# halajun/diasss

Hardware: AMD Instinct MI355X
Metric: sonar frames/sec end-to-end (extract+match+LM solve) (higher is better)
Workload: dtype u8/int32 (extract, match) + f64 (geo gate, LM); 1 GPU; 200 synthetic 2000x1024 frames, dense all-pairs; frames=200, pings=2000, bins=1024, pairs=19900

## Files before the change

### diasss_amd/csrc/dsss_ctx.hip

```cpp
#include "dsss_internal.h"
#include "dsss_pg_sym.h"
#include <algorithm>
#include <chrono>
#include <thread>
#include <atomic>
#include <cstdlib>

void dsss_prof_flush(dsss_ctx* c)
{
    if (!c || c->prof.pending.empty()) return;
    hipStreamSynchronize(c->stream);
    for (const dsss_prof::rec& r : c->prof.pending) {
        float ms = 0;
        if (hipEventElapsedTime(&ms, r.e0, r.e1) == hipSuccess) { c->prof.ms[r.k] += ms; c->prof.launches[r.k] += r.nl; }
        c->prof.pool.push_back(r.e0); c->prof.pool.push_back(r.e1);
    }
    c->prof.pending.clear();
}

dsss_switches dsss_switches_read()
{
    dsss_switches sw;
    if (const char* v = getenv("DSSS_EX_SCRATCH_MB")) sw.ex_scratch_mb = (size_t)std::max(1, atoi(v));
    if (const char* v = getenv("DSSS_EX_UPLOAD_BATCH")) sw.ex_upload_batch = std::max(1, atoi(v));
    sw.ex_verbose = getenv("DSSS_EX_VERBOSE") != nullptr;
    if (const char* v = getenv("DSSS_FS_THREADS")) sw.fs_threads = atoi(v);
    if (const char* v = getenv("DSSS_MT_GRID")) sw.mt_grid = atoi(v) != 0;
    sw.sift_hist_dump = getenv("DSSS_SIFT_HIST_DUMP");
    if (const char* v = getenv("DSSS_REG_PEAKS")) sw.reg_peaks_host = strcmp(v, "host") == 0;
    return sw;
}

extern "C" {

void dsss_mask_params_default(dsss_mask_params* p) { p->factor = 2.5; p->width = 10; p->r = 6; p->side = 150; }
void dsss_orb_params_default(dsss_orb_params* p) { p->nfeatures = 2000; p->scale = 1.2f; p->nlevels = 6; p->ini_th = 12; p->min_th = 7; p->descriptor = DSSS_DESC_ORB; }
void dsss_match_params_default(dsss_match_params* p)
{
    p->use_l2 = 0; p->radius = 8; p->bound_same = 88; p->bound_diff = 80; p->l2_bound = 350; p->ratio = 0.35;
    p->scc_iters = 1000; p->pix_err = 2.5; p->merge_thr = 2.5;
}
void dsss_pg_params_default(dsss_pg_params* p)
{
    p->max_iters = 100; p->rel_tol = 1e-5; p->abs_tol = 1e-5; p->lambda0 = 1e-5; p->lambda_factor = 10;
    p->lambda_max = 1e5; p->min_fidelity = 1e-3; p->add_noise = 1;
}

const char* dsss_strerror(int code)
{
    switch (code) {
    case DSSS_OK: return "ok";
    case DSSS_E_NODEVICE: return "no HIP device (libdsss has no CPU fallback)";
    case DSSS_E_ARG: return "bad argument";
    case DSSS_E_HIP: return "HIP runtime error";
    case DSSS_E_STATE: return "call order violated";
    case DSSS_E_CAPACITY: return "buffer too small";
    case DSSS_E_NUMERIC: return "numerical failure";
    case DSSS_E_COMM: return "communicator / RCCL failure";
    default: return "unknown error";
    }
}
const char* dsss_last_error(const dsss_ctx* c) { return c ? c->err.c_str() : "null context"; }

static int kcap_for(const dsss_orb_params& op) { return ((op.nfeatures + 3 * op.nlevels + 63) / 64 + 1) * 64; }

int dsss_create(int device, int max_frames, dsss_ctx** out)
{
    if (!out || max_frames <= 0) return DSSS_E_ARG;
    int ndev = 0;
    if (hipGetDeviceCount(&ndev) != hipSuccess || ndev <= 0 || device < 0 || device >= ndev) return DSSS_E_NODEVICE;
    if (hipSetDevice(device) != hipSuccess) return DSSS_E_NODEVICE;
    dsss_ctx* c = new dsss_ctx();
    c->device = device;
    dsss_mask_params_default(&c->mp); dsss_orb_params_default(&c->op);
    dsss_match_params_default(&c->mt); dsss_pg_params_default(&c->pg);
    c->max_frames = max_frames;
    c->frames.resize(max_frames);
    c->kcap = kcap_for(c->op);
    if (hipStreamCreateWithFlags(&c->stream, hipStreamNonBlocking) != hipSuccess) { delete c; return DSSS_E_HIP; }
    hipEventCreate(&c->prof.e0); hipEventCreate(&c->prof.e1);
    int prio_lo = 0, prio_hi = 0;
    (void)hipDeviceGetStreamPriorityRange(&prio_lo, &prio_hi);
    for (int i = 0; i < 4; ++i) {
        if (i == 1 && prio_hi != prio_lo) { if (hipStreamCreateWithPriority(&c->xs[i], hipStreamNonBlocking, prio_hi) != hipSuccess) { (void)hipGetLastError(); c->xs[i] = nullptr; } }
        if (!c->xs[i]) hipStreamCreateWithFlags(&c->xs[i], hipStreamNonBlocking);
        hipEventCreateWithFlags(&c->xev[i], hipEventDisableTiming);
    }
    for (int i = 0; i < DSSS_MAX_LEVELS; ++i) { hipEventCreateWithFlags(&c->ex_lev_ev[i], hipEventDisableTiming); hipEventCreateWithFlags(&c->ex_cmp_ev[i], hipEventDisableTiming); }
    for (int i = 0; i < 3; ++i) hipEventCreateWithFlags(&c->ex_side_ev[i], hipEventDisableTiming);
    hipEventCreateWithFlags(&c->xev_main, hipEventDisableTiming);
    *out = c;
    return DSSS_OK;
}

static std::array<dsss_fam_slot, 2> pack_family(dsss_frame& f, size_t pack = 0) { return {{ dsss_slot(f.d_pack, pack * sizeof(double)), dsss_slot(f.h_pack, pack * sizeof(double), DSSS_PINNED) }}; }
static std::array<dsss_fam_slot, 2> gbatch_family(dsss_geo_batch& G, size_t total = 0) { return {{ dsss_slot(G.d, total * sizeof(double)), dsss_slot(G.h, total * sizeof(double), DSSS_PINNED) }}; }
static std::array<dsss_fam_slot, 7> store_family(dsss_ctx* c)
{
    const size_t F = (size_t)c->max_frames, K = (size_t)c->kcap;
    return {{ dsss_slot(c->kps, F * K * sizeof(dsss_kp)), dsss_slot(c->desc, F * K * 32), dsss_slot(c->geo, F * K * 2 * sizeof(double)), dsss_slot(c->nkp_dev, F * sizeof(int)),
              dsss_slot(c->rows_dev, F * sizeof(int)), dsss_slot(c->cols_dev, F * sizeof(int)), dsss_slot(c->bbox_dev, F * 4 * sizeof(double)) }};
}

static void free_frame(dsss_frame& f)
{
    dsss_family_release(f.pack_cap, pack_family(f));
    hipFree(f.mask);
    if (f.pack_ev) hipEventDestroy(f.pack_ev);
    for (int l = 0; l < DSSS_MAX_LEVELS; ++l) hipFree(f.lvl[l]);
    f = dsss_frame();
}

// ... 712 lines not shown
```

### diasss_amd/csrc/dsss_internal.h

```cpp
#pragma once
#include <hip/hip_runtime.h>
#include <cstdint>
#include <cstdio>
#include <cstring>
#include <cmath>
#include <cassert>
#include <array>
#include <string>
#include <utility>
#include <vector>
#include "../../include/dsss.h"

#define DSSS_MAX_LEVELS 8
#define DSSS_PI_REF 3.14159265359

struct dsss_ctx;
int dsss_hip_fail(dsss_ctx* c, hipError_t e, const char* file, int line, const char* call);
int dsss_alloc_fail(dsss_ctx* c, hipError_t e, const char* name, const char* step, size_t bytes);

inline hipError_t dsss_mem_alloc(void** p, size_t bytes, bool pinned) { return pinned ? hipHostMalloc(p, bytes, hipHostMallocDefault) : hipMalloc(p, bytes); }
inline void dsss_mem_free(void* p, bool pinned) { if (p) { if (pinned) (void)hipHostFree(p); else (void)hipFree(p); } }

struct dsss_buf {
    void* p = nullptr; size_t cap = 0; const char* const name; const bool pinned;
// ... 137 lines not shown
    dsss_prof prof;
};

#define DSSS_FAIL(ctx, code, ...) do { char _b[512]; snprintf(_b, sizeof _b, __VA_ARGS__); (ctx)->err = _b; return (code); } while (0)
#define HIPCHK(ctx, call) do { hipError_t _e = (call); if (_e != hipSuccess) return dsss_hip_fail((ctx), _e, __FILE__, __LINE__, #call); } while (0)
inline int dsss_hip_fail(dsss_ctx* c, hipError_t e, const char* file, int line, const char* call)
{
    char b[512]; snprintf(b, sizeof b, "%s:%d %s -> %s", file, line, call, hipGetErrorString(e));
    c->err = b; return DSSS_E_HIP;
}

inline int dsss_alloc_fail(dsss_ctx* c, hipError_t e, const char* name, const char* step, size_t bytes)
{
    char b[512]; snprintf(b, sizeof b, "%s: %s (%zu bytes) -> %s", name, step, bytes, hipGetErrorString(e));
    c->err = b; return DSSS_E_HIP;
}

inline int dsss_buf::reserve(dsss_ctx* c, size_t need_bytes, size_t alloc_bytes)
{
    if (cap >= need_bytes) return DSSS_OK;
    hipError_t e = p ? hipStreamSynchronize(c->stream) : hipSuccess;
    if (e != hipSuccess) { release(); return dsss_alloc_fail(c, e, name, "hipStreamSynchronize before the old block goes", alloc_bytes); }
    release();
    void* q = nullptr;
    if ((e = dsss_mem_alloc(&q, alloc_bytes, pinned)) != hipSuccess) return dsss_alloc_fail(c, e, name, pinned ? "hipHostMalloc" : "hipMalloc", alloc_bytes);
    p = q; cap = alloc_bytes;
    return DSSS_OK;
}
inline int dsss_buf::reserve_keep(dsss_ctx* c, size_t need_bytes, size_t alloc_bytes, size_t keep_bytes)
{
    if (cap >= need_bytes) return DSSS_OK;
    hipError_t e = p ? hipStreamSynchronize(c->stream) : hipSuccess;
    if (e != hipSuccess) return dsss_alloc_fail(c, e, name, "hipStreamSynchronize before the old block goes", alloc_bytes);
    dsss_buf nw(name, pinned);
    if ((e = dsss_mem_alloc(&nw.p, alloc_bytes, pinned)) != hipSuccess) { nw.p = nullptr; return dsss_alloc_fail(c, e, name, pinned ? "hipHostMalloc" : "hipMalloc", alloc_bytes); }
    nw.cap = alloc_bytes;
    if (keep_bytes > 0 && p && (e = hipMemcpy(nw.p, p, keep_bytes, hipMemcpyDeviceToDevice)) != hipSuccess) return dsss_alloc_fail(c, e, name, "copy of the kept prefix", keep_bytes);
    *this = std::move(nw);
    return DSSS_OK;
}
template <class Fam> int dsss_family_alloc(dsss_ctx* c, const char* name, size_t& cap, size_t new_cap, const Fam& fam)
{
    bool any = false;
    for (const dsss_fam_slot& s : fam) any = any || *s.pp != nullptr;
    hipError_t e = any ? hipStreamSynchronize(c->stream) : hipSuccess;
    dsss_family_release(cap, fam);
    if (e != hipSuccess) return dsss_alloc_fail(c, e, name, "hipStreamSynchronize before the old blocks go", 0);
    for (const dsss_fam_slot& s : fam) {
        void* q = nullptr;
        if ((e = dsss_mem_alloc(&q, s.bytes, s.pinned)) != hipSuccess) { dsss_family_release(cap, fam); return dsss_alloc_fail(c, e, name, s.pinned ? "hipHostMalloc" : "hipMalloc", s.bytes); }
        *s.pp = q;
    }
    cap = new_cap;
    return DSSS_OK;
}

struct dsss_scope {
    dsss_ctx* c; int k; int nl; hipEvent_t e0 = nullptr, e1 = nullptr;
    static hipEvent_t take(dsss_ctx* c) {
        hipEvent_t e = nullptr;
        if (!c->prof.pool.empty()) { e = c->prof.pool.back(); c->prof.pool.pop_back(); } else hipEventCreate(&e);
        return e;
    }
    dsss_scope(dsss_ctx* c_, int k_, double work = 0, int launches = 1) : c(c_), k(k_), nl(launches) {
        if (c->prof.on) { c->prof.work[k] += work; e0 = take(c); e1 = take(c); hipEventRecord(e0, c->stream); }
    }
    ~dsss_scope() {
        if (e0) {
            hipEventRecord(e1, c->stream);
            c->prof.pending.push_back({ k, nl, e0, e1 });
            if (c->prof.pending.size() >= 16384) dsss_prof_flush(c);
        }
    }
};

struct dsss_switches {
    size_t ex_scratch_mb = 24576;
    int ex_upload_batch = 8;
    bool ex_verbose = false;
    int fs_threads = 0;
    bool mt_grid = true;
    const char* sift_hist_dump = nullptr;
    bool reg_peaks_host = false;
};
dsss_switches dsss_switches_read();

void dsss_extract_eager(dsss_ctx* c, const int* ids, int n, const dsss_switches& sw);
int dsss_ensure_store(dsss_ctx* c);
int dsss_ensure_sift_store(dsss_ctx* c);
struct ex_frame;
void dsss_launch_sift_desc(dsss_ctx* c, hipStream_t st, const ex_frame* d_exf, int kcap, int nb, const char* hist_dump);
int dsss_frame_geo_bbox(dsss_ctx* c, int id);
int dsss_bboxes_enqueue(dsss_ctx* c);
int dsss_sync_bboxes(dsss_ctx* c);
int dsss_frame_kp_geo(dsss_ctx* c, int id, int n);
int dsss_mt_reserve_pair_index(dsss_ctx* c, size_t npairs);
int dsss_mt_reserve_pair_match(dsss_ctx* c, size_t npairs);
int dsss_mt_reserve_rows(dsss_ctx* c, size_t n);
int dsss_mt_upload_ptr_tables(dsss_ctx* c);
void dsss_mt_clear_results(dsss_ctx* c);
void dsss_mt_free(dsss_ctx* c);
void dsss_pg_free(dsss_ctx* c);
void dsss_comm_free(dsss_ctx* c);
int dsss_comm_rank(const dsss_ctx* c);
int dsss_comm_world(const dsss_ctx* c);
int dsss_comm_allreduce(dsss_ctx* c, double* dev, size_t n, hipStream_t st);
int dsss_comm_allgather(dsss_ctx* c, void* recv_dev, size_t bytes_per_rank, hipStream_t st);

__host__ __device__ inline void dsss_sincos(double x, double* s, double* c)
{
    const double invpio2 = 6.36619772367581382433e-01;
    const double pio2_1 = 1.57079632673412561417e+00;
    const double pio2_1t = 6.07710050650619224932e-11;
    double k = rint(x * invpio2);
    double r = (x - k * pio2_1) - k * pio2_1t;
    double z = r * r;
    double ps = 1.58969099521155010221e-10;
    ps = ps * z + -2.50507602534068634195e-08;
    ps = ps * z + 2.75573137070700676789e-06;
    ps = ps * z + -1.98412698298579493134e-04;
    ps = ps * z + 8.33333333332248946124e-03;
    ps = ps * z + -1.66666666666666324348e-01;
    double sr = r + (r * z) * ps;
    double pc = -1.13596475577881948265e-11;
    pc = pc * z + 2.08757232129817482790e-09;
    pc = pc * z + -2.75573143513906633035e-07;
    pc = pc * z + 2.48015872894767294178e-05;
    pc = pc * z + -1.38888888888741095749e-03;
    pc = pc * z + 4.16666666666666019037e-02;
    double cr = (1.0 - 0.5 * z) + (z * z) * pc;
    long long q = ((long long)k) & 3;
    if (q == 0) { *s = sr; *c = cr; }
    else if (q == 1) { *s = cr; *c = -sr; }
    else if (q == 2) { *s = -sr; *c = -cr; }
    else { *s = -cr; *c = sr; }
}

__host__ __device__ inline void dsss_geo_side(const double* P, bool starboard, double* s, double* c)
{
    dsss_sincos(starboard ? P[2] + DSSS_PI_REF / 2 : P[2] - DSSS_PI_REF / 2, s, c);
}
__host__ __device__ inline int dsss_geo_index(int M, int col)
{
    int half = M / 2, idx;
    if (col >= half) idx = col - half;
    else { idx = half - col; if (idx > half - 1) idx = half - 1; }
    return idx;
}
__host__ __device__ inline void dsss_geo_bin(const double* P, const double* gr, int M, int col, double s, double c, double* x, double* y)
{
    const int idx = dsss_geo_index(M, col);
    *x = (P[3] - 0.0) + gr[idx] * c;
    *y = (P[4] - 0.0) + gr[idx] * s;
}
__host__ __device__ inline void dsss_geo_at(const double* pose6, const double* gr, int M, int row, int col,
                                            double* x, double* y)
{
    const double* P = pose6 + (size_t)row * 6;
    double s, c;
    dsss_geo_side(P, col >= M / 2, &s, &c);
    dsss_geo_bin(P, gr, M, col, s, c, x, y);
}
__host__ __device__ inline void dsss_rotate_row(const double* row, double cx, double cy, double theta, double s, double c, double* out)
{
    out[0] = row[0]; out[1] = row[1]; out[5] = row[5];
    if (theta == 0.0) { out[2] = row[2]; out[3] = row[3]; out[4] = row[4]; return; }
// ... 7 lines not shown
```

### diasss_amd/csrc/dsss_lc.hip

```cpp
#include "dsss_internal.h"
#include "dsss_pose.h"
#include "dsss_lm.h"
#include <algorithm>

#define MR 16
#define MD 15

struct mini_prob {
    pose_t prior, odo;
    double sig_prior[6], sig_odo[6], sig_s[2], sig_t[2];
    double slant_s, slant_t;
};
struct mini_val { double L[3]; pose_t X1, X2; };

#define LG 16
#define LS 16
#define LIDX(i, k) ((k) * LS + (i) + 1)
struct lc_lds { double J[MR * LS]; double H[MD * LS]; double r[MR]; mini_prob m; mini_val v, nv; };

__device__ inline void lc_bcast_pose(const pose_t& mine, int src, pose_t* out)
{
#pragma unroll
    for (int k = 0; k < 9; ++k) out->R[k] = __shfl(mine.R[k], src, LG);
#pragma unroll
    for (int k = 0; k < 3; ++k) out->t[k] = __shfl(mine.t[k], src, LG);
}
__device__ inline void lc_select_pose(bool second, const pose_t& a, const pose_t& b, pose_t* out)
{
#pragma unroll
    for (int k = 0; k < 9; ++k) out->R[k] = second ? b.R[k] : a.R[k];
#pragma unroll
    for (int k = 0; k < 3; ++k) out->t[k] = second ? b.t[k] : a.t[k];
}
__device__ static void mini_lin(const mini_prob& m, const mini_val& v, double* r, double* J, int lane)
{
    const bool hb = (lane & 8) != 0;
    const bool wr = J && (lane & 7) == 0;
    if (J) {
#pragma unroll
        for (int c2 = 0; c2 < LS; ++c2) J[lane * LS + c2] = 0.0;
        __builtin_amdgcn_wave_barrier();
    }
    pose_t t1, t2, E; double xi[6], rr[6];
    const pose_t* P = hb ? &v.X1 : &m.prior;
    const pose_t* Q = hb ? &v.X2 : &v.X1;
    pose_between(P, Q, &t1);
    pose_between(&m.odo, &t1, &t2);
    lc_select_pose(hb, t1, t2, &E);
    pose_log(&E, xi);
#pragma unroll
    for (int i = 0; i < 6; ++i) { const double sg = hb ? m.sig_odo[i] : m.sig_prior[i]; rr[i] = xi[i] / sg; }
    if (!J) {
#pragma unroll
        for (int i = 0; i < 6; ++i) { r[i] = __shfl(rr[i], 0, LG); r[6 + i] = __shfl(rr[i], 8, LG); }
    } else if (wr) {
#pragma unroll
        for (int i = 0; i < 6; ++i) r[(hb ? 6 : 0) + i] = rr[i];
    }
    if (J) {
        pose_t hi; double Ad[36];
        pose_inverse(&t1, &hi);
        pose_adjoint(&hi, Ad);
        if (wr && !hb) {
#pragma unroll
            for (int i = 0; i < 6; ++i) J[i * LS + 3 + i] = 1.0 / m.sig_prior[i];
        }
        if (wr && hb) {
#pragma unroll
            for (int i = 0; i < 6; ++i) {
#pragma unroll
                for (int j = 0; j < 6; ++j) J[(6 + i) * LS + 3 + j] = -Ad[6 * i + j] / m.sig_odo[i];
                J[(6 + i) * LS + 9 + i] = 1.0 / m.sig_odo[i];
            }
        }
    }
    double ee[2], H1[6], H2[12], r2[2];
    const pose_t* X = hb ? &v.X2 : &v.X1;
    const double slant = hb ? m.slant_t : m.slant_s;
    const double sg0 = hb ? m.sig_t[0] : m.sig_s[0], sg1 = hb ? m.sig_t[1] : m.sig_s[1];
    sss_factor(v.L, X, slant, 0.0, ee, J ? H1 : nullptr, H2);
    r2[0] = ee[0] / sg0; r2[1] = ee[1] / sg1;
    if (!J) {
#pragma unroll
        for (int i = 0; i < 2; ++i) { r[12 + i] = __shfl(r2[i], 0, LG); r[14 + i] = __shfl(r2[i], 8, LG); }
    }
    if (wr) {
        const int row0 = hb ? 14 : 12, col0 = hb ? 9 : 3;
        r[row0] = r2[0]; r[row0 + 1] = r2[1];
#pragma unroll
        for (int i = 0; i < 2; ++i) {
            const double sg = i ? sg1 : sg0;
#pragma unroll
            for (int j = 0; j < 3; ++j) J[(row0 + i) * LS + j] = H1[3 * i + j] / sg;
#pragma unroll
            for (int j = 0; j < 6; ++j) J[(row0 + i) * LS + col0 + j] = H2[6 * i + j] / sg;
        }
    }
    if (J) __builtin_amdgcn_wave_barrier();
}
__device__ static __noinline__ double mini_err(const mini_prob& m, const mini_val& v, int lane)
{
    double r[MR];
    mini_lin(m, v, r, nullptr, lane);
    double s = 0;
#pragma unroll
    for (int i = 0; i < MR; ++i) s += r[i] * r[i];
    return 0.5 * s;
}
__device__ static double normal_eq(const double* J, const double* r, double* H, int lane)
{
    double g = 0;
    if (lane < MD) {
        double ca[MR];
#pragma unroll
        for (int k = 0; k < MR; ++k) ca[k] = J[k * LS + lane];
#pragma unroll
        for (int k = 0; k < MR; ++k) g += ca[k] * r[k];
        for (int b2 = 0; b2 < MD; ++b2) {
            double t = 0;
#pragma unroll
            for (int k = 0; k < MR; ++k) t += ca[k] * J[k * LS + b2];
            if (b2 <= lane) H[lane * LS + b2] = t;
            __builtin_amdgcn_sched_barrier(0);
        }
    }
    __builtin_amdgcn_wave_barrier();
    return g;
}
__device__ static int chol15(const double* H, double lambda, double* L, int lane)
{
    double row[MD];
    const int li = lane < MD ? lane : MD - 1;
#pragma unroll
    for (int j = 0; j < MD; ++j) row[j] = j <= li ? H[li * LS + j] + (j == li ? lambda : 0.0) : 0.0;
    int bad = 0;
#pragma unroll
    for (int j = 0; j < MD; ++j) {
        double sacc = row[j];
#pragma unroll
        for (int k = 0; k < MD; ++k) if (k < j) sacc -= row[k] * L[LIDX(j, k)];
        const double dj = __shfl(sacc, j, LG);
        if (!(dj > 0) || !isfinite(dj)) { bad = 1; break; }
        const double dq = sqrt(dj);
        row[j] = li == j ? dq : sacc / dq;
        if (lane < MD && li >= j) L[LIDX(li, j)] = row[j];
        __builtin_amdgcn_wave_barrier();
        __builtin_amdgcn_sched_barrier(0);
    }
    return bad;
}
__device__ static void chol15_solve(const double* L, double* b)
{
#pragma unroll
    for (int i = 0; i < MD; ++i) {
        double sacc = b[i];
#pragma unroll
        for (int k = 0; k < MD; ++k) if (k < i) sacc -= L[LIDX(i, k)] * b[k];
        b[i] = sacc / L[LIDX(i, i)];
        __builtin_amdgcn_sched_barrier(0);
    }
#pragma unroll
    for (int i = MD - 1; i >= 0; --i) {
        double sacc = b[i];
#pragma unroll
        for (int k = 0; k < MD; ++k) if (k > i) sacc -= L[LIDX(k, i)] * b[k];
        b[i] = sacc / L[LIDX(i, i)];
        __builtin_amdgcn_sched_barrier(0);
    }
}

__device__ inline void lc_comp_pose(bool on, pose_t* C)
{
    const double flipv[3] = { 0, 0, DSSS_PI_REF };
    pose_identity(C); if (on) so3_exp(flipv, C->R);
}
__device__ inline void lc_sss_sigmas(double slant, double* sig) { sig[0] = 0.1; sig[1] = slant * (0.1 * DSSS_PI_REF / 180); }
__device__ inline void lc_landmark_start(const double* geo_s, const double* geo_t, double z_s, double alt_s, double z_t, double alt_t, double* L)
{
    L[0] = (geo_s[0] + geo_t[0]) / 2; L[1] = (geo_s[1] + geo_t[1]) / 2; L[2] = ((z_s - alt_s) + (z_t - alt_t)) / 2;
}

struct lc_tables { const double* const* __restrict__ alt; const double* const* __restrict__ gr; const double* const* __restrict__ pose; const int* __restrict__ cols; };
static lc_tables lc_tables_of(const dsss_ctx* c) { const int F = c->max_frames; return { c->d_ptrs, c->d_ptrs + F, c->d_ptrs + 2 * F, c->cols_dev }; }

__device__ inline void lc_setup(lc_lds& S, const lc_tables& T, const double* kp, int fs, int ft, int flip, int lane, double* geo)
{
    const double PI = DSSS_PI_REF;
    const double* pose_s = T.pose[fs]; const double* pose_t_ = T.pose[ft];
    const int id_s = (int)kp[0], id_t = (int)kp[3];
    const bool hb = (lane & 8) != 0;
    mini_prob m;
    m.slant_s = kp[2]; m.slant_t = kp[5]; lc_sss_sigmas(kp[2], m.sig_s); lc_sss_sigmas(kp[5], m.sig_t);
    pose_t Tp_s, Tp_t, Tp_st;
    {
        pose_t Pm, Cm, Tm;
        pose_from_rodrigues(hb ? pose_t_ + (size_t)id_t * 6 : pose_s + (size_t)id_s * 6, &Pm);
        lc_comp_pose(flip & (hb ? 2 : 1), &Cm);
        pose_compose(&Pm, &Cm, &Tm);
        lc_bcast_pose(Tm, 0, &Tp_s); lc_bcast_pose(Tm, 8, &Tp_t);
    }
    pose_between(&Tp_s, &Tp_t, &Tp_st);
    for (int k = 0; k < 6; ++k) m.sig_prior[k] = 0.000001;
    m.sig_odo[0] = 0.1 * PI / 180; m.sig_odo[1] = 0.1 * PI / 180; m.sig_odo[2] = 0.5 * PI / 180;
    m.sig_odo[3] = fabs(Tp_st.t[0] * 2); m.sig_odo[4] = fabs(Tp_st.t[1] / 10); m.sig_odo[5] = 0.1;
    for (int k = 3; k < 5; ++k) if (m.sig_odo[k] < 1e-9) m.sig_odo[k] = 1e-9;
    m.prior = Tp_s; m.odo = Tp_st;
    double gx, gy;
    dsss_geo_at(hb ? pose_t_ : pose_s, hb ? T.gr[ft] : T.gr[fs], hb ? T.cols[ft] : T.cols[fs], hb ? id_t : id_s, hb ? (int)kp[4] : (int)kp[1], &gx, &gy);
    geo[0] = __shfl(gx, 0, LG); geo[1] = __shfl(gy, 0, LG); geo[2] = __shfl(gx, 8, LG); geo[3] = __shfl(gy, 8, LG);
    mini_val v;
    lc_landmark_start(geo, geo + 2, pose_s[(size_t)id_s * 6 + 5], T.alt[fs][id_s], pose_t_[(size_t)id_t * 6 + 5], T.alt[ft][id_t], v.L);
    v.X1 = Tp_s; v.X2 = Tp_t;
    if (lane == 0) { S.m = m; S.v = v; }
    __builtin_amdgcn_wave_barrier();
}
__device__ inline lm_verdict lc_trial(lc_lds& S, const lm_rule& R, double g_mine, double lambda, double oldLin, double err, int lane, double* newErr)
{
    const lm_verdict refused = { false, false };
    if (chol15(S.H, lambda, S.H, lane) != 0) return refused;
    double d[MD];
#pragma unroll
    for (int a = 0; a < MD; ++a) d[a] = -__shfl(g_mine, a, LG);
    chol15_solve(S.H, d);
    double sk = S.r[lane];
#pragma unroll
    for (int a = 0; a < MD; ++a) sk += S.J[lane * LS + a] * d[a];
    double newLin = 0;
#pragma unroll
    for (int k = 0; k < MR; ++k) { const double t = __shfl(sk, k, LG); newLin += t * t; }
    newLin *= 0.5;
    if (!lm_descends(oldLin, newLin)) return refused;
    {
        const bool hb = (lane & 8) != 0;
        pose_t Xn; double dx[6];
        const pose_t* X = hb ? &S.v.X2 : &S.v.X1;
#pragma unroll
        for (int a = 0; a < 6; ++a) dx[a] = hb ? d[9 + a] : d[3 + a];
        pose_retract(X, dx, &Xn);
        if (lane == 0) { for (int a = 0; a < 3; ++a) S.nv.L[a] = S.v.L[a] + d[a]; S.nv.X1 = Xn; }
        if (lane == 8) S.nv.X2 = Xn;
        __builtin_amdgcn_wave_barrier();
    }
    *newErr = mini_err(S.m, S.nv, lane);
    return lm_judge(R, oldLin, newLin, err, *newErr);
}
__device__ inline void lc_take_trial(lc_lds& S, int lane)
{
    const double* src = reinterpret_cast<const double*>(&S.nv); double* dst = reinterpret_cast<double*>(&S.v);
    const double e0 = src[lane], e1 = lane + LG < (int)(sizeof(mini_val) / sizeof(double)) ? src[lane + LG] : 0.0;
    __builtin_amdgcn_wave_barrier();
    dst[lane] = e0; if (lane + LG < (int)(sizeof(mini_val) / sizeof(double))) dst[lane + LG] = e1;
    __builtin_amdgcn_wave_barrier();
}
__device__ inline int lc_lm(lc_lds& S, int lane, double* err_io)
{
    const lm_rule R = lm_gtsam_defaults();
    double lambda = 1e-5, err = *err_io, cur;
    int iters = 0;
    if (err > 0) do {
        cur = err;
        mini_lin(S.m, S.v, S.r, S.J, lane);
        const double g_mine = normal_eq(S.J, S.r, S.H, lane);
        double oldLin = 0;
#pragma unroll
        for (int k = 0; k < MR; ++k) oldLin += S.r[k] * S.r[k];
        oldLin *= 0.5;
        for (;;) {
            double newErr = 0;
            const lm_verdict v = lc_trial(S, R, g_mine, lambda, oldLin, err, lane, &newErr);
            if (v.success) { lc_take_trial(S, lane); err = newErr; lm_accepted(R, &lambda); ++iters; break; }
            if (v.stop || lm_refused(R, &lambda)) break;
        }
    } while (lm_continue(R, iters, cur, err));
    *err_io = err; return iters;
}
__device__ inline double lc_score(const lc_lds& S, const double* kp, const double* gr_t, int Mt, int flip, const double* geo, pose_t* new_pose)
{
    const double PI = DSSS_PI_REF;
    pose_t cq, cti;
    lc_comp_pose(flip & 2, &cq); pose_inverse(&cq, &cti);
    pose_compose(&S.v.X2, &cti, new_pose);
    const double x_o = geo[0] - geo[2], y_o = geo[1] - geo[3], ini = sqrt(x_o * x_o + y_o * y_o);
    double rpy[3]; pose_rpy(new_pose, rpy);
    const bool port = kp[4] < Mt / 2;
    const int gi = port ? Mt / 2 - (int)kp[4] : (int)kp[4] - Mt / 2;
    const double bearing = port ? rpy[2] + PI / 2 - PI : rpy[2] - PI / 2 - PI;
    const double lx = new_pose->t[0] + gr_t[gi] * cos(bearing), ly = new_pose->t[1] + gr_t[gi] * sin(bearing);
    const double x_n = geo[0] - lx, y_n = geo[1] - ly;
    return ini / sqrt(x_n * x_n + y_n * y_n) - 2;
}
__device__ inline void lc_marginal_var(lc_lds& S, int lane, double* var)
{
    mini_lin(S.m, S.v, S.r, S.J, lane);
    (void)normal_eq(S.J, S.r, S.H, lane);
    double var_mine = NAN;
    if (chol15(S.H, 0.0, S.H, lane) == 0) {
        double d[MD];
#pragma unroll
        for (int a = 0; a < MD; ++a) d[a] = (a == 9 + lane) ? 1.0 : 0.0;
        chol15_solve(S.H, d);
        var_mine = 0;
#pragma unroll
        for (int a = 9; a < MD; ++a) if (a == 9 + lane) var_mine = d[a];
    }
#pragma unroll
    for (int c2 = 0; c2 < 6; ++c2) var[c2] = __shfl(var_mine, c2, LG);
}
__device__ inline void lc_rel_pose(const lc_lds& S, int flip, const pose_t& new_pose, double* rel12)
{
    pose_t cq, csi, src, rel;
    lc_comp_pose(flip & 1, &cq); pose_inverse(&cq, &csi);
    pose_compose(&S.m.prior, &csi, &src); pose_between(&src, &new_pose, &rel);
    for (int a = 0; a < 9; ++a) rel12[a] = rel.R[a];
    for (int a = 0; a < 3; ++a) rel12[9 + a] = rel.t[a];
}

__global__ __launch_bounds__(64, 2) void lc_kernel(const double* __restrict__ kp7, int n, const int* __restrict__ kp7_pair, const uint8_t* __restrict__ kp7_flip,
                                                const int* __restrict__ act_s, const int* __restrict__ act_t, int single_s, int single_t, lc_tables T, dsss_lc* __restrict__ out)
{
    __shared__ lc_lds s_all[64 / LG];
    const int grp = threadIdx.x / LG, lane = threadIdx.x % LG;
    const int i = blockIdx.x * (64 / LG) + grp;
    if (i >= n) return;
    lc_lds& S = s_all[grp];
    const double* kp = kp7 + (size_t)i * 7;
    const int fs = kp7_pair ? act_s[kp7_pair[i]] : single_s, ft = kp7_pair ? act_t[kp7_pair[i]] : single_t;
    const int flip = kp7_flip[i];
    double geo[4]; dsss_lc o;
    lc_setup(S, T, kp, fs, ft, flip, lane, geo);
    o.pad_ = 0; o.err0 = o.err1 = mini_err(S.m, S.v, lane);
    o.iters = lc_lm(S, lane, &o.err1);
    pose_t new_pose;
    o.score = lc_score(S, kp, T.gr[ft], T.cols[ft], flip, geo, &new_pose);
    lc_marginal_var(S, lane, o.var);
    lc_rel_pose(S, flip, new_pose, o.rel);
    if (lane == 0) out[i] = o;
}

struct tri_frame { const double* pose; const double* alt; const double* gr; int M; };
struct tri_prob { pose_t Tp_s, Tp_t; double slant_s, slant_t, sig_s[2], sig_t[2], sig_p[3], ini[3]; };

__device__ inline void tri_setup(tri_prob& P, const double* kp, const tri_frame& s, const tri_frame& t, int flip, const double* q)
{
    if (q) {
        for (int k = 0; k < 9; ++k) { P.Tp_s.R[k] = q[k]; P.Tp_t.R[k] = q[12 + k]; }
        for (int k = 0; k < 3; ++k) { P.Tp_s.t[k] = q[9 + k]; P.Tp_t.t[k] = q[21 + k]; P.ini[k] = q[24 + k]; }
    } else {
        const int id_s = (int)kp[0], id_t = (int)kp[3];
        pose_t cps_s, cps_t, Ps, Pt;
        lc_comp_pose(flip & 1, &cps_s); lc_comp_pose(flip & 2, &cps_t);
        pose_from_rodrigues(s.pose + (size_t)id_s * 6, &Ps); pose_from_rodrigues(t.pose + (size_t)id_t * 6, &Pt);
        pose_compose(&Ps, &cps_s, &P.Tp_s); pose_compose(&Pt, &cps_t, &P.Tp_t);
        double geo_s[2], geo_t[2];
        dsss_geo_at(s.pose, s.gr, s.M, id_s, (int)kp[1], &geo_s[0], &geo_s[1]);
        dsss_geo_at(t.pose, t.gr, t.M, id_t, (int)kp[4], &geo_t[0], &geo_t[1]);
        lc_landmark_start(geo_s, geo_t, s.pose[(size_t)id_s * 6 + 5], s.alt[id_s], t.pose[(size_t)id_t * 6 + 5], t.alt[id_t], P.ini);
    }
    P.slant_s = kp[2]; P.slant_t = kp[5]; lc_sss_sigmas(kp[2], P.sig_s); lc_sss_sigmas(kp[5], P.sig_t);
    const double dx = P.Tp_s.t[0] - P.Tp_t.t[0], dy = P.Tp_s.t[1] - P.Tp_t.t[1];
    P.sig_p[0] = 10.0; P.sig_p[1] = 10.0; P.sig_p[2] = sqrt(dx * dx + dy * dy) / 100;
    if (P.sig_p[2] < 1e-9) P.sig_p[2] = 1e-9;
}
__device__ static void tri_lin(const tri_prob& P, const double* p, double* r, double* J)
{
    double ee[2], H1[6], H2[12];
    sss_factor(p, &P.Tp_s, P.slant_s, 0.0, ee, J ? H1 : nullptr, H2);
    for (int i = 0; i < 2; ++i) { r[i] = ee[i] / P.sig_s[i]; if (J) for (int j = 0; j < 3; ++j) J[i * 3 + j] = H1[3 * i + j] / P.sig_s[i]; }
    sss_factor(p, &P.Tp_t, P.slant_t, 0.0, ee, J ? H1 : nullptr, H2);
    for (int i = 0; i < 2; ++i) { r[2 + i] = ee[i] / P.sig_t[i]; if (J) for (int j = 0; j < 3; ++j) J[(2 + i) * 3 + j] = H1[3 * i + j] / P.sig_t[i]; }
    for (int i = 0; i < 3; ++i) { r[4 + i] = (p[i] - P.ini[i]) / P.sig_p[i]; if (J) for (int j = 0; j < 3; ++j) J[(4 + i) * 3 + j] = (i == j) ? 1.0 / P.sig_p[i] : 0.0; }
}
__device__ static double tri_err(const tri_prob& P, const double* p)
{
    double rr[7], t = 0;
    tri_lin(P, p, rr, nullptr); for (int k = 0; k < 7; ++k) t += rr[k] * rr[k];
    return 0.5 * t;
}
__device__ static int tri_chol3(double* A)
{
    for (int j = 0; j < 3; ++j) {
        double d = A[j * 3 + j];
        for (int k = 0; k < j; ++k) d -= A[j * 3 + k] * A[j * 3 + k];
        if (!(d > 0) || !isfinite(d)) return -1;
        d = sqrt(d); A[j * 3 + j] = d;
        for (int i = j + 1; i < 3; ++i) { double t = A[i * 3 + j]; for (int k = 0; k < j; ++k) t -= A[i * 3 + k] * A[j * 3 + k]; A[i * 3 + j] = t / d; }
    }
    return 0;
}
__device__ inline void tri_lm(const tri_prob& P, double* p)
{
    const lm_rule R = lm_gtsam_defaults();
    double lambda = 1e-5, err = tri_err(P, p), cur;
    int iters = 0;
    if (err > 0) do {
        cur = err;
        double r[7], J[21], H[9], g[3];
        tri_lin(P, p, r, J);
        for (int a = 0; a < 3; ++a) {
            double t = 0; for (int k = 0; k < 7; ++k) t += J[k * 3 + a] * r[k];
            g[a] = t;
            for (int b = 0; b < 3; ++b) { double u = 0; for (int k = 0; k < 7; ++k) u += J[k * 3 + a] * J[k * 3 + b]; H[a * 3 + b] = u; }
        }
        double oldLin = 0; for (int k = 0; k < 7; ++k) oldLin += r[k] * r[k];
        oldLin *= 0.5;
        for (;;) {
            double A[9], d[3], np_[3] = { 0, 0, 0 }, newErr = 0, newLin = 0;
            lm_verdict v = { false, false };
            for (int a = 0; a < 9; ++a) A[a] = H[a];
            for (int a = 0; a < 3; ++a) { A[a * 3 + a] += lambda; d[a] = -g[a]; }
            if (tri_chol3(A) == 0) {
                for (int a = 0; a < 3; ++a) { double t = d[a]; for (int k = 0; k < a; ++k) t -= A[a * 3 + k] * d[k]; d[a] = t / A[a * 3 + a]; }
                for (int a = 2; a >= 0; --a) { double t = d[a]; for (int k = a + 1; k < 3; ++k) t -= A[k * 3 + a] * d[k]; d[a] = t / A[a * 3 + a]; }
                for (int k = 0; k < 7; ++k) { double t = r[k]; for (int a = 0; a < 3; ++a) t += J[k * 3 + a] * d[a]; newLin += t * t; }
                newLin *= 0.5;
                if (lm_descends(oldLin, newLin)) {
                    for (int a = 0; a < 3; ++a) np_[a] = p[a] + d[a];
                    newErr = tri_err(P, np_);
                    v = lm_judge(R, oldLin, newLin, err, newErr);
                }
            }
            if (v.success) { for (int a = 0; a < 3; ++a) p[a] = np_[a]; err = newErr; lm_accepted(R, &lambda); ++iters; break; }
            if (v.stop || lm_refused(R, &lambda)) break;
        }
    } while (lm_continue(R, iters, cur, err));
}
__global__ __launch_bounds__(64) void tri_kernel(const double* __restrict__ kp7, int n, const uint8_t* __restrict__ flips, tri_frame fs, tri_frame ft,
                                                 const double* __restrict__ explicit27, double* __restrict__ out7)
{
    const int i = blockIdx.x * 64 + threadIdx.x;
    if (i >= n) return;
    const double* kp = kp7 + (size_t)i * 7;
    tri_prob P;
    tri_setup(P, kp, fs, ft, flips ? flips[i] : 0, explicit27 ? explicit27 + (size_t)i * 27 : nullptr);
    double p[3] = { P.ini[0], P.ini[1], P.ini[2] };
    tri_lm(P, p);
    double* o = out7 + (size_t)i * 7;
    o[0] = p[0]; o[1] = p[1]; o[2] = p[2];
    double e[2];
    sss_factor(p, &P.Tp_s, P.slant_s, 0.0, e, nullptr, nullptr); o[3] = fabs(e[0]); o[4] = fabs(e[1]);
    sss_factor(p, &P.Tp_t, P.slant_t, 0.0, e, nullptr, nullptr); o[5] = fabs(e[0]); o[6] = fabs(e[1]);
}

static int check_kp7_rows(dsss_ctx* c, const dsss_frame& fs, const dsss_frame& ft, const double* rows, int n, int pair)
{
    for (int i = 0; i < n; ++i) {
        const double* k = rows + (size_t)i * 7;
        if (k[0] >= 0 && k[0] < fs.N && k[3] >= 0 && k[3] < ft.N && k[1] >= 1 && k[1] < fs.M && k[4] >= 1 && k[4] < ft.M) continue;
        char who[32] = ""; if (pair >= 0) snprintf(who, sizeof who, "pair %d ", pair);
        DSSS_FAIL(c, DSSS_E_ARG, "%skp7 row %d: ping/bin outside the frames (%g,%g | %g,%g)", who, i, k[0], k[1], k[3], k[4]);
    }
    return DSSS_OK;
}
static void lc_sticky_flags(const dsss_frame& fs, const dsss_frame& ft, const double* rows, int n, uint8_t* flip)
{
    uint8_t f = 0;
    for (int i = 0; i < n; ++i) {
        const double* k = rows + (size_t)i * 7;
        if (dsss_yaw_flips(fs.h_geo[(size_t)(int)k[0] * 6 + 2])) f |= 1;
        if (dsss_yaw_flips(ft.h_geo[(size_t)(int)k[3] * 6 + 2])) f |= 2;
        flip[i] = f;
    }
}
static int lc_one_list(dsss_ctx* c, int id_s, int id_t, const double* kp7, int n, std::vector<double>* h, std::vector<uint8_t>* flip)
{
    if (id_s < 0 || id_s >= c->max_frames || id_t < 0 || id_t >= c->max_frames) DSSS_FAIL(c, DSSS_E_ARG, "frame id out of range");
    const dsss_frame &fs = c->frames[id_s], &ft = c->frames[id_t];
    if (!fs.has_geom || !ft.has_geom) DSSS_FAIL(c, DSSS_E_STATE, "frames need dsss_frame_set first");
    if (!fs.h_geo || !ft.h_geo) DSSS_FAIL(c, DSSS_E_STATE, "host copy of the DR poses missing");
    if (n == 0) return DSSS_OK;
    HIPCHK(c, hipSetDevice(c->device));
    h->resize((size_t)n * 7); flip->resize(n);
    HIPCHK(c, hipMemcpy(h->data(), kp7, h->size() * sizeof(double), hipMemcpyDefault));
    if (const int rc = check_kp7_rows(c, fs, ft, h->data(), n, -1)) return rc;
    lc_sticky_flags(fs, ft, h->data(), n, flip->data());
    return DSSS_OK;
}
static int lc_launch(dsss_ctx* c, const double* kp7, int n, const int* kp7_pair, const uint8_t* kp7_flip, const int* act_s, const int* act_t, int single_s, int single_t,
                     dsss_lc* out)
{
    dsss_scope sc(c, DSSS_K_LC);
    hipLaunchKernelGGL(lc_kernel, dim3((n + 3) / 4), dim3(64), 0, c->stream, kp7, n, kp7_pair, kp7_flip, act_s, act_t, single_s, single_t, lc_tables_of(c), out);
    HIPCHK(c, hipGetLastError());
    return DSSS_OK;
}
static int tri_run(dsss_ctx* c, const double* kp7, int n, const uint8_t* h_flip, const tri_frame& fs, const tri_frame& ft, const double* in27, double* out7)
{
    const size_t nd = (size_t)n * (7 + 7 + (in27 ? 27 : 0));
    dsss_buf d("triangulation rows, inputs and results");
    if (const int rc = d.reserve(c, nd * sizeof(double) + (h_flip ? (size_t)n : 0))) return rc;
    double* d_kp7 = d.as<double>(); double* d_out = d_kp7 + (size_t)n * 7; double* d_in = in27 ? d_out + (size_t)n * 7 : nullptr;
    uint8_t* d_flip = h_flip ? reinterpret_cast<uint8_t*>(d_kp7 + nd) : nullptr;
    HIPCHK(c, hipMemcpyAsync(d_kp7, kp7, (size_t)n * 7 * sizeof(double), hipMemcpyDefault, c->stream));
    if (d_in) HIPCHK(c, hipMemcpyAsync(d_in, in27, (size_t)n * 27 * sizeof(double), hipMemcpyDefault, c->stream));
    if (d_flip) HIPCHK(c, hipMemcpyAsync(d_flip, h_flip, (size_t)n, hipMemcpyHostToDevice, c->stream));
    hipLaunchKernelGGL(tri_kernel, dim3((n + 63) / 64), dim3(64), 0, c->stream, (const double*)d_kp7, n, (const uint8_t*)d_flip, fs, ft, (const double*)d_in, d_out);
    HIPCHK(c, hipGetLastError());
    HIPCHK(c, hipMemcpyAsync(out7, d_out, (size_t)n * 7 * sizeof(double), hipMemcpyDeviceToHost, c->stream));
    HIPCHK(c, hipStreamSynchronize(c->stream));
    return DSSS_OK;
}
static tri_frame tri_frame_of(const dsss_frame& f) { return { f.pose6, f.alt, f.gr, f.M }; }

extern "C" {

int dsss_lc_solve_all(dsss_ctx* c)
{
    if (!c) return DSSS_E_ARG;
    HIPCHK(c, hipSetDevice(c->device));
    const int n = c->total_kp7;
    c->has_lc = false;
    if (const int rc = c->lcs.reserve(c, (size_t)n * sizeof(dsss_lc), ((size_t)n + 1024) * sizeof(dsss_lc))) return rc;
    if (n > 0)
        if (const int rc = lc_launch(c, c->kp7, n, c->kp7_pair, c->kp7_flip, c->act_s, c->act_t, 0, 0, c->lcs.as<dsss_lc>())) return rc;
    c->has_lc = true; ++c->lc_gen;
    return DSSS_OK;
}

int dsss_lc_get(dsss_ctx* c, int pair, dsss_lc* out, int cap, int* nout)
{
    if (!c) return DSSS_E_ARG;
    if (pair < 0 || pair >= c->npairs) DSSS_FAIL(c, DSSS_E_ARG, "pair %d out of range", pair);
    if (!c->has_lc) DSSS_FAIL(c, DSSS_E_STATE, "dsss_lc_solve_all has not run");
    const int a = c->pair_active[pair];
    const int n = a < 0 ? 0 : c->h_kp7_off[a + 1] - c->h_kp7_off[a];
    if (nout) *nout = n;
    if (n == 0 || !out) return DSSS_OK;
    if (cap < n) DSSS_FAIL(c, DSSS_E_CAPACITY, "caller capacity %d < %d", cap, n);
    HIPCHK(c, hipStreamSynchronize(c->stream));
    HIPCHK(c, hipMemcpy(out, c->lcs.as<dsss_lc>() + c->h_kp7_off[a], (size_t)n * sizeof(dsss_lc), hipMemcpyDeviceToHost));
    return DSSS_OK;
}

int dsss_lc_solve_pairs(dsss_ctx* c, const int* src_ids, const int* tgt_ids, int npairs, const double* kp7, const int* pair_off)
{
    if (!c || npairs < 0 || (npairs > 0 && (!src_ids || !tgt_ids || !pair_off))) return DSSS_E_ARG;
    dsss_mt_clear_results(c);
    HIPCHK(c, hipSetDevice(c->device));
    const int n = npairs > 0 ? pair_off[npairs] : 0;
    if (n < 0 || (n > 0 && !kp7)) return DSSS_E_ARG;
    for (int p = 0; p < npairs; ++p) {
        const int s = src_ids[p], t = tgt_ids[p];
        if (s < 0 || s >= c->max_frames || t < 0 || t >= c->max_frames || s == t) DSSS_FAIL(c, DSSS_E_ARG, "pair %d: bad frame ids (%d,%d)", p, s, t);
        if (!c->frames[s].has_geom || !c->frames[t].has_geom) DSSS_FAIL(c, DSSS_E_STATE, "pair %d: frames need dsss_frame_set first", p);
        if (pair_off[p + 1] < pair_off[p] || pair_off[0] != 0) DSSS_FAIL(c, DSSS_E_ARG, "pair_off does not start at 0 or is not ascending at pair %d", p);
    }
    int rc = dsss_sync_bboxes(c); if (rc) return rc;
    if ((rc = dsss_mt_upload_ptr_tables(c))) return rc;
    std::vector<double> h((size_t)n * 7);
    if (n > 0) HIPCHK(c, hipMemcpy(h.data(), kp7, h.size() * sizeof(double), hipMemcpyDefault));
    std::vector<int> h_pair(n); std::vector<uint8_t> h_flip(n);
    for (int p = 0; p < npairs && n > 0; ++p) {
        const dsss_frame &fs = c->frames[src_ids[p]], &ft = c->frames[tgt_ids[p]];
        const int o = pair_off[p], np = pair_off[p + 1] - o;
        if (!fs.h_geo || !ft.h_geo) DSSS_FAIL(c, DSSS_E_STATE, "pair %d: host copy of the DR poses missing", p);
        if ((rc = check_kp7_rows(c, fs, ft, h.data() + (size_t)o * 7, np, p))) return rc;
        lc_sticky_flags(fs, ft, h.data() + (size_t)o * 7, np, h_flip.data() + o);
        std::fill(h_pair.begin() + o, h_pair.begin() + o + np, p);
    }
    if (n > 0) {
        HIPCHK(c, hipStreamSynchronize(c->stream));
        if ((rc = dsss_mt_reserve_pair_index(c, npairs)) || (rc = dsss_mt_reserve_rows(c, n))) return rc;
        HIPCHK(c, hipMemcpy(c->act_s, src_ids, npairs * sizeof(int), hipMemcpyHostToDevice)); HIPCHK(c, hipMemcpy(c->act_t, tgt_ids, npairs * sizeof(int), hipMemcpyHostToDevice));
        HIPCHK(c, hipMemcpy(c->kp7_off, pair_off, (npairs + 1) * sizeof(int), hipMemcpyHostToDevice));
        HIPCHK(c, hipMemcpy(c->kp7, h.data(), h.size() * sizeof(double), hipMemcpyHostToDevice));
        HIPCHK(c, hipMemcpy(c->kp7_pair, h_pair.data(), (size_t)n * sizeof(int), hipMemcpyHostToDevice)); HIPCHK(c, hipMemcpy(c->kp7_flip, h_flip.data(), (size_t)n, hipMemcpyHostToDevice));
    }
    c->npairs = c->nactive = npairs; c->total_kp7 = n;
    c->pair_s.assign(src_ids, src_ids + npairs); c->pair_t.assign(tgt_ids, tgt_ids + npairs);
    c->pair_active.resize(npairs); for (int p = 0; p < npairs; ++p) c->pair_active[p] = p;
    c->h_row_off.assign(npairs + 1, 0); if (npairs > 0) c->h_kp7_off.assign(pair_off, pair_off + npairs + 1);
    return dsss_lc_solve_all(c);
}

int dsss_lc_solve(dsss_ctx* c, int id_s, int id_t, const double* kp7, int n, dsss_lc* out)
{
    if (!c || n < 0 || (n > 0 && (!kp7 || !out))) return DSSS_E_ARG;
    std::vector<double> h; std::vector<uint8_t> flip;
    int rc = lc_one_list(c, id_s, id_t, kp7, n, &h, &flip); if (rc || n == 0) return rc;
    if ((rc = dsss_sync_bboxes(c))) return rc;
    if ((rc = dsss_mt_upload_ptr_tables(c))) return rc;
    dsss_buf d_kp7("dsss_lc_solve kp7"), d_flip("dsss_lc_solve flags"), d_out("dsss_lc_solve results");
    if ((rc = d_kp7.reserve(c, h.size() * sizeof(double))) || (rc = d_flip.reserve(c, flip.size())) || (rc = d_out.reserve(c, (size_t)n * sizeof(dsss_lc)))) return rc;
    HIPCHK(c, hipMemcpyAsync(d_kp7.p, h.data(), h.size() * sizeof(double), hipMemcpyHostToDevice, c->stream));
    HIPCHK(c, hipMemcpyAsync(d_flip.p, flip.data(), flip.size(), hipMemcpyHostToDevice, c->stream));
    if ((rc = lc_launch(c, d_kp7.as<double>(), n, nullptr, d_flip.as<uint8_t>(), nullptr, nullptr, id_s, id_t, d_out.as<dsss_lc>()))) return rc;
    HIPCHK(c, hipMemcpyAsync(out, d_out.p, (size_t)n * sizeof(dsss_lc), hipMemcpyDeviceToHost, c->stream));
    HIPCHK(c, hipStreamSynchronize(c->stream));
    return DSSS_OK;
}

int dsss_triangulate(dsss_ctx* c, int id_s, int id_t, const double* kp7, int n, double* out7)
{
    if (!c || n < 0 || (n > 0 && (!kp7 || !out7))) return DSSS_E_ARG;
    std::vector<double> h; std::vector<uint8_t> flip;
    const int rc = lc_one_list(c, id_s, id_t, kp7, n, &h, &flip); if (rc || n == 0) return rc;
    return tri_run(c, h.data(), n, flip.data(), tri_frame_of(c->frames[id_s]), tri_frame_of(c->frames[id_t]), nullptr, out7);
}

int dsss_triangulate_poses(dsss_ctx* c, const double* kp7, const double* in27, int n, double* out7)
{
    if (!c || n < 0 || (n > 0 && (!kp7 || !in27 || !out7))) return DSSS_E_ARG;
    if (n == 0) return DSSS_OK;
    HIPCHK(c, hipSetDevice(c->device));
    return tri_run(c, kp7, n, nullptr, tri_frame{}, tri_frame{}, in27, out7);
}

}
```

Baseline: 9687 frames/s.

## Reuse linearization across LM iterations in loop-closure mini-solver

The per-keypoint LM solver no longer relinearizes unconditionally at the top of each iteration. When a trial step is expected to be accepted (the linear decrease is large), it computes the full Jacobian at the trial point instead of only the error, and the next iteration and the marginal-variance step reuse it. It also zeroes the Jacobian once at setup rather than on every linearization, and spreads the Jacobian row writes across lanes instead of one writer lane per half. The old behaviour stays available behind DSSS_LC_RELIN. The risk is wasted Jacobian work on predicted-accepted trials that end up rejected, plus more code size in the kernel.

```diff
diff --git a/diasss_amd/csrc/dsss_ctx.hip b/diasss_amd/csrc/dsss_ctx.hip
--- a/diasss_amd/csrc/dsss_ctx.hip
+++ b/diasss_amd/csrc/dsss_ctx.hip
@@ -28,6 +28,7 @@
     if (const char* v = getenv("DSSS_MT_GRID")) sw.mt_grid = atoi(v) != 0;
     sw.sift_hist_dump = getenv("DSSS_SIFT_HIST_DUMP");
     if (const char* v = getenv("DSSS_REG_PEAKS")) sw.reg_peaks_host = strcmp(v, "host") == 0;
+    if (const char* v = getenv("DSSS_LC_RELIN")) sw.lc_relin = atoi(v) != 0;
     return sw;
 }
 
diff --git a/diasss_amd/csrc/dsss_internal.h b/diasss_amd/csrc/dsss_internal.h
--- a/diasss_amd/csrc/dsss_internal.h
+++ b/diasss_amd/csrc/dsss_internal.h
@@ -243,6 +243,7 @@
     bool mt_grid = true;
     const char* sift_hist_dump = nullptr;
     bool reg_peaks_host = false;
+    bool lc_relin = false;
 };
 dsss_switches dsss_switches_read();
 
diff --git a/diasss_amd/csrc/dsss_lc.hip b/diasss_amd/csrc/dsss_lc.hip
--- a/diasss_amd/csrc/dsss_lc.hip
+++ b/diasss_amd/csrc/dsss_lc.hip
@@ -32,15 +32,10 @@
 #pragma unroll
     for (int k = 0; k < 3; ++k) out->t[k] = second ? b.t[k] : a.t[k];
 }
-__device__ static void mini_lin(const mini_prob& m, const mini_val& v, double* r, double* J, int lane)
+__device__ __forceinline__ void mini_lin_body(const mini_prob& m, const mini_val& v, double* r, double* J, int lane)
 {
     const bool hb = (lane & 8) != 0;
     const bool wr = J && (lane & 7) == 0;
-    if (J) {
-#pragma unroll
-        for (int c2 = 0; c2 < LS; ++c2) J[lane * LS + c2] = 0.0;
-        __builtin_amdgcn_wave_barrier();
-    }
     pose_t t1, t2, E; double xi[6], rr[6];
     const pose_t* P = hb ? &v.X1 : &m.prior;
     const pose_t* Q = hb ? &v.X2 : &v.X1;
@@ -61,17 +56,18 @@
         pose_t hi; double Ad[36];
         pose_inverse(&t1, &hi);
         pose_adjoint(&hi, Ad);
-        if (wr && !hb) {
-#pragma unroll
-            for (int i = 0; i < 6; ++i) J[i * LS + 3 + i] = 1.0 / m.sig_prior[i];
-        }
-        if (wr && hb) {
-#pragma unroll
-            for (int i = 0; i < 6; ++i) {
-#pragma unroll
-                for (int j = 0; j < 6; ++j) J[(6 + i) * LS + 3 + j] = -Ad[6 * i + j] / m.sig_odo[i];
-                J[(6 + i) * LS + 9 + i] = 1.0 / m.sig_odo[i];
+        const int q = lane & 7;
+        if (q < 6 && !hb) J[q * LS + 3 + q] = 1.0 / m.sig_prior[q];
+        if (q < 6 && hb) {
+            const double sg = m.sig_odo[q];
+#pragma unroll
+            for (int j = 0; j < 6; ++j) {
+                double a = Ad[j];
+#pragma unroll
+                for (int i = 1; i < 6; ++i) a = q == i ? Ad[6 * i + j] : a;
+                J[(6 + q) * LS + 3 + j] = -a / sg;
             }
+            J[(6 + q) * LS + 9 + q] = 1.0 / sg;
         }
     }
     double ee[2], H1[6], H2[12], r2[2];
@@ -84,28 +80,30 @@
 #pragma unroll
         for (int i = 0; i < 2; ++i) { r[12 + i] = __shfl(r2[i], 0, LG); r[14 + i] = __shfl(r2[i], 8, LG); }
     }
-    if (wr) {
-        const int row0 = hb ? 14 : 12, col0 = hb ? 9 : 3;
-        r[row0] = r2[0]; r[row0 + 1] = r2[1];
-#pragma unroll
-        for (int i = 0; i < 2; ++i) {
-            const double sg = i ? sg1 : sg0;
-#pragma unroll
-            for (int j = 0; j < 3; ++j) J[(row0 + i) * LS + j] = H1[3 * i + j] / sg;
-#pragma unroll
-            for (int j = 0; j < 6; ++j) J[(row0 + i) * LS + col0 + j] = H2[6 * i + j] / sg;
-        }
+    if (wr) { const int row0 = hb ? 14 : 12; r[row0] = r2[0]; r[row0 + 1] = r2[1]; }
+    if (J && (lane & 7) < 2) {
+        const int i = lane & 7, row = (hb ? 14 : 12) + i, col0 = hb ? 9 : 3;
+        const double sg = i ? sg1 : sg0;
+#pragma unroll
+        for (int j = 0; j < 3; ++j) J[row * LS + j] = (i ? H1[3 + j] : H1[j]) / sg;
+#pragma unroll
+        for (int j = 0; j < 6; ++j) J[row * LS + col0 + j] = (i ? H2[6 + j] : H2[j]) / sg;
     }
     if (J) __builtin_amdgcn_wave_barrier();
 }
+__device__ inline double lc_half_sq(const double* r)
+{
+    double s = 0;
+#pragma unroll
+    for (int k = 0; k < MR; ++k) s += r[k] * r[k];
+    return 0.5 * s;
+}
+__device__ static __noinline__ void mini_lin(const mini_prob& m, const mini_val& v, double* r, double* J, int lane) { mini_lin_body(m, v, r, J, lane); }
 __device__ static __noinline__ double mini_err(const mini_prob& m, const mini_val& v, int lane)
 {
     double r[MR];
-    mini_lin(m, v, r, nullptr, lane);
-    double s = 0;
-#pragma unroll
-    for (int i = 0; i < MR; ++i) s += r[i] * r[i];
-    return 0.5 * s;
+    mini_lin_body(m, v, r, nullptr, lane);
+    return lc_half_sq(r);
 }
 __device__ static double normal_eq(const double* J, const double* r, double* H, int lane)
 {
@@ -212,12 +210,22 @@
     lc_landmark_start(geo, geo + 2, pose_s[(size_t)id_s * 6 + 5], T.alt[fs][id_s], pose_t_[(size_t)id_t * 6 + 5], T.alt[ft][id_t], v.L);
     v.X1 = Tp_s; v.X2 = Tp_t;
     if (lane == 0) { S.m = m; S.v = v; }
+#pragma unroll
+    for (int c2 = 0; c2 < LS; ++c2) S.J[lane * LS + c2] = 0.0;
     __builtin_amdgcn_wave_barrier();
 }
-__device__ inline lm_verdict lc_trial(lc_lds& S, const lm_rule& R, double g_mine, double lambda, double oldLin, double err, int lane, double* newErr)
-{
+__device__ inline void lc_lin_at_v(lc_lds& S, int lane, bool* at_v)
+{
+    if (!*at_v) { mini_lin(S.m, S.v, S.r, S.J, lane); *at_v = true; }
+}
+__device__ inline bool lc_lin_with_trial(const lm_rule& R, double oldLin, double newLin, double err) { return oldLin - newLin > 100 * R.relTol * err; }
+template <bool RELIN>
+__device__ inline lm_verdict lc_trial(lc_lds& S, const lm_rule& R, double g_mine, double lambda, double oldLin, double err, int lane, bool* at_v, bool* at_nv, double* newErr)
+{
+    *at_nv = false;
     const lm_verdict refused = { false, false };
     if (chol15(S.H, lambda, S.H, lane) != 0) return refused;
+    lc_lin_at_v(S, lane, at_v);
     double d[MD];
 #pragma unroll
     for (int a = 0; a < MD; ++a) d[a] = -__shfl(g_mine, a, LG);
@@ -241,7 +249,11 @@
         if (lane == 8) S.nv.X2 = Xn;
         __builtin_amdgcn_wave_barrier();
     }
-    *newErr = mini_err(S.m, S.nv, lane);
+    if (!RELIN && lc_lin_with_trial(R, oldLin, newLin, err)) {
+        mini_lin(S.m, S.nv, S.r, S.J, lane); *at_v = false; *at_nv = true;
+        *newErr = lc_half_sq(S.r);
+    } else
+        *newErr = mini_err(S.m, S.nv, lane);
     return lm_judge(R, oldLin, newLin, err, *newErr);
 }
 __device__ inline void lc_take_trial(lc_lds& S, int lane)
@@ -252,23 +264,21 @@
     dst[lane] = e0; if (lane + LG < (int)(sizeof(mini_val) / sizeof(double))) dst[lane + LG] = e1;
     __builtin_amdgcn_wave_barrier();
 }
-__device__ inline int lc_lm(lc_lds& S, int lane, double* err_io)
+template <bool RELIN> __device__ inline int lc_lm(lc_lds& S, int lane, bool* at_v, double* err_io)
 {
     const lm_rule R = lm_gtsam_defaults();
     double lambda = 1e-5, err = *err_io, cur;
     int iters = 0;
     if (err > 0) do {
         cur = err;
-        mini_lin(S.m, S.v, S.r, S.J, lane);
+        if (RELIN) *at_v = false;
+        lc_lin_at_v(S, lane, at_v);
         const double g_mine = normal_eq(S.J, S.r, S.H, lane);
-        double oldLin = 0;
-#pragma unroll
-        for (int k = 0; k < MR; ++k) oldLin += S.r[k] * S.r[k];
-        oldLin *= 0.5;
+        const double oldLin = lc_half_sq(S.r);
         for (;;) {
-            double newErr = 0;
-            const lm_verdict v = lc_trial(S, R, g_mine, lambda, oldLin, err, lane, &newErr);
-            if (v.success) { lc_take_trial(S, lane); err = newErr; lm_accepted(R, &lambda); ++iters; break; }
+            double newErr = 0; bool at_nv;
+            const lm_verdict v = lc_trial<RELIN>(S, R, g_mine, lambda, oldLin, err, lane, at_v, &at_nv, &newErr);
+            if (v.success) { lc_take_trial(S, lane); *at_v = at_nv; err = newErr; lm_accepted(R, &lambda); ++iters; break; }
             if (v.stop || lm_refused(R, &lambda)) break;
         }
     } while (lm_continue(R, iters, cur, err));
@@ -289,9 +299,9 @@
     const double x_n = geo[0] - lx, y_n = geo[1] - ly;
     return ini / sqrt(x_n * x_n + y_n * y_n) - 2;
 }
-__device__ inline void lc_marginal_var(lc_lds& S, int lane, double* var)
-{
-    mini_lin(S.m, S.v, S.r, S.J, lane);
+__device__ inline void lc_marginal_var(lc_lds& S, int lane, bool* at_v, double* var)
+{
+    lc_lin_at_v(S, lane, at_v);
     (void)normal_eq(S.J, S.r, S.H, lane);
     double var_mine = NAN;
     if (chol15(S.H, 0.0, S.H, lane) == 0) {
@@ -315,6 +325,7 @@
     for (int a = 0; a < 3; ++a) rel12[9 + a] = rel.t[a];
 }
 
+template <bool RELIN>
 __global__ __launch_bounds__(64, 2) void lc_kernel(const double* __restrict__ kp7, int n, const int* __restrict__ kp7_pair, const uint8_t* __restrict__ kp7_flip,
                                                 const int* __restrict__ act_s, const int* __restrict__ act_t, int single_s, int single_t, lc_tables T, dsss_lc* __restrict__ out)
 {
@@ -328,11 +339,14 @@
     const int flip = kp7_flip[i];
     double geo[4]; dsss_lc o;
     lc_setup(S, T, kp, fs, ft, flip, lane, geo);
-    o.pad_ = 0; o.err0 = o.err1 = mini_err(S.m, S.v, lane);
-    o.iters = lc_lm(S, lane, &o.err1);
+    mini_lin(S.m, S.v, S.r, S.J, lane);
+    bool at_v = true;
+    o.pad_ = 0; o.err0 = o.err1 = lc_half_sq(S.r);
+    o.iters = lc_lm<RELIN>(S, lane, &at_v, &o.err1);
     pose_t new_pose;
     o.score = lc_score(S, kp, T.gr[ft], T.cols[ft], flip, geo, &new_pose);
-    lc_marginal_var(S, lane, o.var);
+    if (RELIN) at_v = false;
+    lc_marginal_var(S, lane, &at_v, o.var);
     lc_rel_pose(S, flip, new_pose, o.rel);
     if (lane == 0) out[i] = o;
 }
@@ -475,11 +489,12 @@
     lc_sticky_flags(fs, ft, h->data(), n, flip->data());
     return DSSS_OK;
 }
-static int lc_launch(dsss_ctx* c, const double* kp7, int n, const int* kp7_pair, const uint8_t* kp7_flip, const int* act_s, const int* act_t, int single_s, int single_t,
-                     dsss_lc* out)
+static int lc_launch(dsss_ctx* c, bool relin, const double* kp7, int n, const int* kp7_pair, const uint8_t* kp7_flip, const int* act_s, const int* act_t, int single_s,
+                     int single_t, dsss_lc* out)
 {
     dsss_scope sc(c, DSSS_K_LC);
-    hipLaunchKernelGGL(lc_kernel, dim3((n + 3) / 4), dim3(64), 0, c->stream, kp7, n, kp7_pair, kp7_flip, act_s, act_t, single_s, single_t, lc_tables_of(c), out);
+    hipLaunchKernelGGL(relin ? lc_kernel<true> : lc_kernel<false>, dim3((n + 3) / 4), dim3(64), 0, c->stream, kp7, n, kp7_pair, kp7_flip, act_s, act_t, single_s, single_t,
+                       lc_tables_of(c), out);
     HIPCHK(c, hipGetLastError());
     return DSSS_OK;
 }
@@ -511,7 +526,7 @@
     c->has_lc = false;
     if (const int rc = c->lcs.reserve(c, (size_t)n * sizeof(dsss_lc), ((size_t)n + 1024) * sizeof(dsss_lc))) return rc;
     if (n > 0)
-        if (const int rc = lc_launch(c, c->kp7, n, c->kp7_pair, c->kp7_flip, c->act_s, c->act_t, 0, 0, c->lcs.as<dsss_lc>())) return rc;
+        if (const int rc = lc_launch(c, dsss_switches_read().lc_relin, c->kp7, n, c->kp7_pair, c->kp7_flip, c->act_s, c->act_t, 0, 0, c->lcs.as<dsss_lc>())) return rc;
     c->has_lc = true; ++c->lc_gen;
     return DSSS_OK;
 }
@@ -583,7 +598,7 @@
     if ((rc = d_kp7.reserve(c, h.size() * sizeof(double))) || (rc = d_flip.reserve(c, flip.size())) || (rc = d_out.reserve(c, (size_t)n * sizeof(dsss_lc)))) return rc;
     HIPCHK(c, hipMemcpyAsync(d_kp7.p, h.data(), h.size() * sizeof(double), hipMemcpyHostToDevice, c->stream));
     HIPCHK(c, hipMemcpyAsync(d_flip.p, flip.data(), flip.size(), hipMemcpyHostToDevice, c->stream));
-    if ((rc = lc_launch(c, d_kp7.as<double>(), n, nullptr, d_flip.as<uint8_t>(), nullptr, nullptr, id_s, id_t, d_out.as<dsss_lc>()))) return rc;
+    if ((rc = lc_launch(c, dsss_switches_read().lc_relin, d_kp7.as<double>(), n, nullptr, d_flip.as<uint8_t>(), nullptr, nullptr, id_s, id_t, d_out.as<dsss_lc>()))) return rc;
     HIPCHK(c, hipMemcpyAsync(out, d_out.p, (size_t)n * sizeof(dsss_lc), hipMemcpyDeviceToHost, c->stream));
     HIPCHK(c, hipStreamSynchronize(c->stream));
     return DSSS_OK;
```

New measurement: 9639 frames/s. No clear change (-0.5%).
